# nelilepo/timetabling-ga-mpi-openmp

Hardware: AMD Instinct MI355X
Metric: fitness evals/sec (hcv+scv), pop 64K, 400-event instance; 1/2/4/8 GPUs (higher is better)
Workload: dtype i32; 1 GPU; med instance E=400 R=10 F=5 S=200 (seeded synthetic, medium01-size), population 65536 per GPU, one tt_eval (hcv+scv+feasible+penalty) per step; pop_per_gpu=65536, global_pop=65536, kernel=eval_tile5_w8, parallelism=dp1 (independent population shards)

## Files before the change

### timetabling-ga-mpi-openmp_amd/csrc/tt_eval.hip

```cpp
#include <algorithm>
#include <type_traits>
#include <utility>
#include <vector>

#include "tt_internal.h"

namespace ttga {

typedef __attribute__((address_space(4))) const uint32_t ConstU32;
typedef __attribute__((address_space(4))) const int32_t ConstI32;


__device__ __forceinline__ int bcnt_acc(uint32_t x, int acc) {
    int r;
    asm("v_bcnt_u32_b32 %0, %1, %2" : "=v"(r) : "v"(x), "v"(acc));
    return r;
}
__device__ __forceinline__ int popc_acc(uint64_t x, int acc) {
    int r, t;
    asm("v_bcnt_u32_b32 %0, %1, %2" : "=v"(t) : "v"((uint32_t)x), "v"(acc));
    asm("v_bcnt_u32_b32 %0, %1, %2" : "=v"(r) : "v"((uint32_t)(x >> 32)), "v"(t));
    return r;
}

__device__ __forceinline__ uint32_t lds_addr(const void* p) {
    return (uint32_t)(uintptr_t)(const __attribute__((address_space(3))) void*)p;
}
#define TT_RD(k, o) "ds_read_b64 %" #k ", %" #o " offset:" #k "*8\n"
template <int N>
__device__ __forceinline__ void lds_row_b64(uint32_t addr, uint64_t* v) {
    static_assert(N >= 1 && N <= 7, "1..7 words");
    uint64_t d[7];
    if constexpr (N == 7)
        asm volatile(TT_RD(0, 7) TT_RD(1, 7) TT_RD(2, 7) TT_RD(3, 7) TT_RD(4, 7) TT_RD(5, 7) TT_RD(6, 7) "s_waitcnt lgkmcnt(0)"
                     : "=&v"(d[0]), "=&v"(d[1]), "=&v"(d[2]), "=&v"(d[3]), "=&v"(d[4]), "=&v"(d[5]), "=&v"(d[6])
                     : "v"(addr) : "memory");
    else if constexpr (N == 6)
        asm volatile(TT_RD(0, 6) TT_RD(1, 6) TT_RD(2, 6) TT_RD(3, 6) TT_RD(4, 6) TT_RD(5, 6) "s_waitcnt lgkmcnt(0)"
                     : "=&v"(d[0]), "=&v"(d[1]), "=&v"(d[2]), "=&v"(d[3]), "=&v"(d[4]), "=&v"(d[5]) : "v"(addr) : "memory");
    else if constexpr (N == 5)
        asm volatile(TT_RD(0, 5) TT_RD(1, 5) TT_RD(2, 5) TT_RD(3, 5) TT_RD(4, 5) "s_waitcnt lgkmcnt(0)"
                     : "=&v"(d[0]), "=&v"(d[1]), "=&v"(d[2]), "=&v"(d[3]), "=&v"(d[4]) : "v"(addr) : "memory");
    else if constexpr (N == 4)
        asm volatile(TT_RD(0, 4) TT_RD(1, 4) TT_RD(2, 4) TT_RD(3, 4) "s_waitcnt lgkmcnt(0)"
                     : "=&v"(d[0]), "=&v"(d[1]), "=&v"(d[2]), "=&v"(d[3]) : "v"(addr) : "memory");
    else if constexpr (N == 3)
        asm volatile(TT_RD(0, 3) TT_RD(1, 3) TT_RD(2, 3) "s_waitcnt lgkmcnt(0)"
                     : "=&v"(d[0]), "=&v"(d[1]), "=&v"(d[2]) : "v"(addr) : "memory");
    else if constexpr (N == 2)
        asm volatile(TT_RD(0, 2) TT_RD(1, 2) "s_waitcnt lgkmcnt(0)" : "=&v"(d[0]), "=&v"(d[1]) : "v"(addr) : "memory");
    else
        asm volatile(TT_RD(0, 1) "s_waitcnt lgkmcnt(0)" : "=&v"(d[0]) : "v"(addr) : "memory");
#pragma unroll
    for (int k = 0; k < N; ++k) v[k] = d[k];
}
#undef TT_RD

#define TT_O(k) [d##k] "=&v"(d[k])
#define TT_I(k) [x##k] "v"(k < NA ? a : b), [o##k] "i"(k < NA ? 8 * k : 8 * (k - NA))
#define TT_R(k) "ds_read_b64 %[d" #k "], %[x" #k "] offset:%[o" #k "]\n"
template <int NA, int NB>
__device__ __forceinline__ void lds_two_rows(uint32_t a, uint32_t b, uint64_t* v) {
    constexpr int N = NA + NB;
    static_assert(NA >= 1 && NB >= 0 && N <= 8, "1..8 words");
    uint64_t d[8];
    if constexpr (N == 8)
        asm volatile(TT_R(0) TT_R(1) TT_R(2) TT_R(3) TT_R(4) TT_R(5) TT_R(6) TT_R(7) "s_waitcnt lgkmcnt(0)"
                     : TT_O(0), TT_O(1), TT_O(2), TT_O(3), TT_O(4), TT_O(5), TT_O(6), TT_O(7)
                     : TT_I(0), TT_I(1), TT_I(2), TT_I(3), TT_I(4), TT_I(5), TT_I(6), TT_I(7) : "memory");
    else if constexpr (N == 7)
        asm volatile(TT_R(0) TT_R(1) TT_R(2) TT_R(3) TT_R(4) TT_R(5) TT_R(6) "s_waitcnt lgkmcnt(0)"
                     : TT_O(0), TT_O(1), TT_O(2), TT_O(3), TT_O(4), TT_O(5), TT_O(6)
                     : TT_I(0), TT_I(1), TT_I(2), TT_I(3), TT_I(4), TT_I(5), TT_I(6) : "memory");
    else if constexpr (N == 6)
        asm volatile(TT_R(0) TT_R(1) TT_R(2) TT_R(3) TT_R(4) TT_R(5) "s_waitcnt lgkmcnt(0)"
                     : TT_O(0), TT_O(1), TT_O(2), TT_O(3), TT_O(4), TT_O(5)
                     : TT_I(0), TT_I(1), TT_I(2), TT_I(3), TT_I(4), TT_I(5) : "memory");
    else if constexpr (N == 5)
        asm volatile(TT_R(0) TT_R(1) TT_R(2) TT_R(3) TT_R(4) "s_waitcnt lgkmcnt(0)"
                     : TT_O(0), TT_O(1), TT_O(2), TT_O(3), TT_O(4) : TT_I(0), TT_I(1), TT_I(2), TT_I(3), TT_I(4) : "memory");
    else if constexpr (N == 4)
        asm volatile(TT_R(0) TT_R(1) TT_R(2) TT_R(3) "s_waitcnt lgkmcnt(0)"
                     : TT_O(0), TT_O(1), TT_O(2), TT_O(3) : TT_I(0), TT_I(1), TT_I(2), TT_I(3) : "memory");
    else if constexpr (N == 3)
        asm volatile(TT_R(0) TT_R(1) TT_R(2) "s_waitcnt lgkmcnt(0)"
                     : TT_O(0), TT_O(1), TT_O(2) : TT_I(0), TT_I(1), TT_I(2) : "memory");
    else if constexpr (N == 2)
        asm volatile(TT_R(0) TT_R(1) "s_waitcnt lgkmcnt(0)" : TT_O(0), TT_O(1) : TT_I(0), TT_I(1) : "memory");
    else
        asm volatile(TT_R(0) "s_waitcnt lgkmcnt(0)" : TT_O(0) : TT_I(0) : "memory");
#pragma unroll
    for (int k = 0; k < N; ++k) v[k] = d[k];
}
#undef TT_O
#undef TT_I
#undef TT_R

template <int R, int EWC>
__device__ __forceinline__ void corr_words(uint32_t bbase, const uint32_t* sv, const uint64_t (*cup)[EWC], int lane,
                                           int E, bool last_partial, int& h) {
    constexpr int S = EWC - 1 - R;
    if constexpr (R < S) {
        const uint32_t ss = (S < EWC - 1 || !last_partial || lane + 64 * S < E) ? sv[S] : 0u;
        uint64_t bw[EWC + 1];
        lds_two_rows<EWC - R, EWC - S>(bbase + sv[R] * (uint32_t)(EWC * 8) + 8 * R,
                                       bbase + ss * (uint32_t)(EWC * 8) + 8 * S, bw);
#pragma unroll
        for (int w = R; w < EWC; ++w) h = popc_acc(cup[R][w] & bw[w - R], h);
#pragma unroll
        for (int w = S; w < EWC; ++w) h = popc_acc(cup[S][w] & bw[EWC - R + w - S], h);
        corr_words<R + 1, EWC>(bbase, sv, cup, lane, E, last_partial, h);
    } else if constexpr (R == S) {
        if (R < EWC - 1 || !last_partial || lane + 64 * R < E) {
            uint64_t bw[EWC - R];
            lds_row_b64<EWC - R>(bbase + sv[R] * (uint32_t)(EWC * 8) + 8 * R, bw);
#pragma unroll
            for (int w = R; w < EWC; ++w) h = popc_acc(cup[R][w] & bw[w - R], h);
        }
    }
}

template <int ST>
__device__ __forceinline__ void sload_rec(const ConstU32* q, uint32_t (&r)[ST]) {
#pragma unroll
    for (int j = 0; j < ST; ++j) r[j] = q[j];
}
template <int ST>
__device__ __forceinline__ void keep_rec(const uint32_t (&r)[ST]) {
#pragma unroll
    for (int j = 0; j < ST; ++j) asm volatile("" ::"s"(r[j]));
}

constexpr uint32_t kGapLoK = 0x1FF7FDFFu, kGapLoG = 0x20080200u;
constexpr uint32_t kGapHiK = 0x0007FDFFu, kGapHiG = 0x00080200u;
__device__ __forceinline__ int mask_scv_gap(uint64_t m) {
    int sc = __popcll(m & (m >> 1) & (m >> 2));
    const uint32_t lo = (uint32_t)m, hi = (uint32_t)(m >> 32);
    const uint32_t blo = lo + kGapLoK, bhi = hi + kGapHiK;
    const uint32_t tlo = (lo & blo) + kGapLoK, thi = (hi & bhi) + kGapHiK;
    sc += __popc((blo ^ tlo) & kGapLoG);
    sc += __popc((bhi ^ thi) & kGapHiG);
    return sc;
}
__device__ __forceinline__ uint32_t gap_slots4(uint32_t x) {
    const uint32_t o = x | 0x80808080u;
    const uint32_t g9 = ((o - 0x09090909u) >> 7) & 0x01010101u, g18 = ((o - 0x12121212u) >> 7) & 0x01010101u;
    const uint32_t g27 = ((o - 0x1B1B1B1Bu) >> 7) & 0x01010101u, g36 = ((o - 0x24242424u) >> 7) & 0x01010101u;
    return x + g9 + g18 + g36 + 3u * g27;
}
__device__ __forceinline__ uint8_t gap_slot(uint32_t s) { return (uint8_t)gap_slots4(s); }
template <bool GAP>
__device__ __forceinline__ int mask_terms(uint64_t m) { return GAP ? mask_scv_gap(m) : mask_scv(m); }
template <int N, int K, bool GAP = false>
__device__ __forceinline__ int students_scv(const uint8_t* my, const uint32_t* r) {
    constexpr int H = N / 2;
    uint32_t sl[K * N];
#pragma unroll
    for (int k = 0; k < K; ++k)
#pragma unroll
        for (int j = 0; j < N; ++j) sl[k * N + j] = my[(r[k * H + (j >> 1)] >> (16 * (j & 1))) & 0xFFFFu];
    int sc = 0;
#pragma unroll
    for (int k = 0; k < K; ++k) {
        uint64_t m = 0;
#pragma unroll
        for (int j = 0; j < N; ++j) m |= 1ull << (sl[k * N + j] & 63);
        sc += mask_terms<GAP>(m);
    }
    return sc;
}
template <int N, int KMAX, bool GAP = false>
__device__ __forceinline__ int run_scv(const uint8_t* my, const uint32_t* p, int cnt) {
    constexpr int K = N <= 16 ? KMAX : 1;
    constexpr int ST = K * N / 2;
    const int steps = cnt / K;
    int sc = 0;
    if constexpr (KMAX == 1) {
        const ConstU32* q = (const ConstU32*)p;
        uint32_t cur[N / 2];
#pragma unroll
        for (int j = 0; j < N / 2; ++j) cur[j] = q[j];
        for (int i = 0; i < cnt; ++i) {
            const int in = i + 1 < cnt ? i + 1 : i;
            uint32_t nxt[N / 2];
#pragma unroll
            for (int j = 0; j < N / 2; ++j) nxt[j] = q[in * (N / 2) + j];
            uint32_t sl[N];
#pragma unroll
            for (int j = 0; j < N; ++j) sl[j] = my[(cur[j >> 1] >> (16 * (j & 1))) & 0xFFFFu];
            uint64_t m = 0;
#pragma unroll
            for (int j = 0; j < N; ++j) m |= 1ull << (sl[j] & 63);
            sc += mask_terms<GAP>(m);
#pragma unroll
            for (int j = 0; j < N / 2; ++j) cur[j] = nxt[j];
        }
        return sc;
    }
    const ConstU32* q = (const ConstU32*)p;
    if (steps > 0) {
        int i = 0;
        uint32_t ra[ST], rb[ST];
        sload_rec<ST>(q, ra);
        while (true) {
            sload_rec<ST>(q + (i + 1 < steps ? i + 1 : i) * ST, rb);
            sc += students_scv<N, K, GAP>(my, ra);
            keep_rec<ST>(rb);
            if (++i == steps) break;
            sload_rec<ST>(q + (i + 1 < steps ? i + 1 : i) * ST, ra);
            sc += students_scv<N, K, GAP>(my, rb);
            keep_rec<ST>(ra);
            if (++i == steps) break;
        }
    }
    if constexpr (K == 2) {
        if (cnt & 1) {
            uint32_t r[N / 2];
            sload_rec<N / 2>(q + steps * ST, r);
            sc += students_scv<N, 1, GAP>(my, r);
        }
    }
    return sc;
}
__device__ __noinline__ int run_scv_any(const uint8_t* my, const ConstU32* p, int cnt, int n, bool gap) {
    int sc = 0;
    for (int i = 0; i < cnt; ++i) {
        uint64_t m = 0;
        for (int j = 0; j < n / 2; ++j) {
            const uint32_t d = p[i * (n / 2) + j];
            m |= 1ull << (my[d & 0xFFFFu] & 63);
            m |= 1ull << (my[d >> 16] & 63);
        }
        sc += gap ? mask_scv_gap(m) : mask_scv(m);
    }
    return sc;
}
template <int KMAX, bool GAP = false>
__device__ __forceinline__ int lane_scv_runs(const uint8_t* my, const DevProblem& pb, int r0, int r1) {
    const ConstI32* runs = (const ConstI32*)pb.srun;
    int sc = 0;
    for (int k = r0; k < r1; ++k) {
        const int n = runs[4 * k], off = runs[4 * k + 1], cnt = runs[4 * k + 2];
        const uint32_t* p = pb.sid + off;
        switch (n) {
#define TT_RUN(N) case N: sc += run_scv<N, KMAX, GAP>(my, p, cnt); break;
            TT_RUN(2) TT_RUN(4) TT_RUN(6) TT_RUN(8) TT_RUN(10) TT_RUN(12) TT_RUN(14) TT_RUN(16)
            TT_RUN(18) TT_RUN(20) TT_RUN(22) TT_RUN(24) TT_RUN(26) TT_RUN(28) TT_RUN(30) TT_RUN(32)
#undef TT_RUN
            default: sc += run_scv_any(my, (const ConstU32*)p, cnt, n, GAP); break;
        }
    }
    return sc;
}

#ifndef TT_EVAL_ABLATE
#define TT_EVAL_ABLATE 0
#endif
__host__ __device__ inline int t5_cnt_bytes(int R) {
    return kSlots * ((R + 1) / 2) * 4;
}

struct Tile5Layout {
    int SP, WS;
    size_t tile_bytes, off_ws, off_part, bytes;
};

__host__ __device__ inline Tile5Layout tile5_layout(int E, int R, int NW, bool DB = false) {
    Tile5Layout L;
    int sp = (E + 1 + 3) & ~3;
    if (((sp >> 2) & 1) == 0) sp += 4;
    L.SP = sp;
    const int ew64 = (E + 63) / 64;
    const int cntb = t5_cnt_bytes(R);
    L.WS = (kSlots * ew64 * 8 + cntb + 15) & ~15;
    L.tile_bytes = ((size_t)64 * sp + 15) & ~(size_t)15;
    L.off_ws = (DB ? 2 : 1) * L.tile_bytes;
    L.off_part = L.off_ws + (size_t)NW * L.WS;
    L.bytes = L.off_part + 4 * (size_t)(NW * 64 + 64);
    return L;
}

template <int NW>
__device__ __forceinline__ void tile_dma(const uint8_t* src, uint8_t* dst, int np, int E, int SP, int wv, int lane) {
    const int qd = E >> 2;
    const __amdgpu_buffer_rsrc_t rs = __builtin_amdgcn_make_buffer_rsrc((void*)src, 0, np * E, 0x00020000);
    for (int r = wv; r < np; r += NW) {
        if (lane < qd)
            __builtin_amdgcn_raw_ptr_buffer_load_lds(rs, (__attribute__((address_space(3))) void*)(dst + r * SP), 4,
                                                     4 * lane, r * E, 0, 0);
        if (lane + 64 < qd)
            __builtin_amdgcn_raw_ptr_buffer_load_lds(rs, (__attribute__((address_space(3))) void*)(dst + r * SP + 256),
                                                     4, 4 * lane + 256, r * E, 0, 0);
    }
}

#ifdef TT_T5_STAMP
constexpr int kT5Launches = 8, kT5MaxBlocks = 16384, kT5Words = 10;
__device__ unsigned long long g_t5_stamp[kT5Launches * kT5MaxBlocks * kT5Words];
#endif

__device__ __forceinline__ uint32_t mad_u16_hi(uint32_t a, uint32_t b, uint32_t c) {
    uint32_t d;
    asm("v_mad_u32_u16 %0, %1, %2, %3 op_sel:[0,1,0,0]" : "=v"(d) : "v"(a), "v"(b), "v"(c));
    return d;
}

constexpr int kT5PrioLane = 3;
constexpr uint32_t kT5PrioW = 0x00112233u;
template <int EWC, int NW, int PK, bool DB = false>
__global__ __launch_bounds__(64 * NW, 4) void eval_tile5_kernel(DevProblem pb, const uint8_t* __restrict__ slot,
                                                              const uint8_t* __restrict__ room, int P,
                                                              int32_t* __restrict__ hcv_out,
                                                              int32_t* __restrict__ scv_out,
                                                              uint8_t* __restrict__ feas_out,
                                                              int32_t* __restrict__ pen_out, int ablate_arg) {
    extern __shared__ __attribute__((aligned(16))) uint8_t lds[];
    const int ablate = TT_EVAL_ABLATE ? ablate_arg : (ablate_arg & 3);
    constexpr int NT = 64 * NW;
#ifdef TT_T5_STAMP
    unsigned long long* st_rec =
        g_t5_stamp + ((size_t)((ablate_arg >> 8) & (kT5Launches - 1)) * kT5MaxBlocks + (blockIdx.x % kT5MaxBlocks)) * kT5Words;
    if (threadIdx.x == 0) {
        const unsigned long long t0 = __builtin_amdgcn_s_memrealtime();
        unsigned hw, xcc;
        asm volatile("s_getreg_b32 %0, hwreg(HW_REG_HW_ID)" : "=s"(hw));
        asm volatile("s_getreg_b32 %0, hwreg(HW_REG_XCC_ID)" : "=s"(xcc));
        st_rec[0] = t0;
        st_rec[1] = ((unsigned long long)xcc << 32) | hw;
    }
#endif
    const int E = pb.E, R = pb.R;
    const int lane = threadIdx.x & 63, wv = wave_id();
    const Tile5Layout L = tile5_layout(E, R, NW, DB);
    const int SP = L.SP;
    uint8_t* tile = lds;
    uint8_t* ws = lds + L.off_ws + (size_t)wv * L.WS;
    uint64_t* B = (uint64_t*)ws;
    uint32_t* cnt = (uint32_t*)(B + kSlots * EWC);
    int32_t* part = (int32_t*)(lds + L.off_part);
    int32_t* hq = part + NW * 64;
    const int tiles = (P + 63) / 64;
    const bool last_partial = E < 64 * EWC;
    const int RW = (R + 1) / 2;

    using PossT = typename std::conditional<PK == 0, uint64_t, uint32_t>::type;
    uint64_t inv_cup[EWC][EWC];
    PossT inv_poss[EWC];
    uint32_t inv_ps[EWC];
    int inv_sn[EWC];
#pragma unroll
    for (int r = 0; r < EWC; ++r) {
        const int e = lane + 64 * r;
        const bool ok = e < E;
        if constexpr (PK == 1) {
            inv_ps[r] = ok ? ((~(uint32_t)pb.poss[e] & 0xFFFFu) | ((uint32_t)pb.sn[e] << 16)) : 0u;
        } else {
            inv_poss[r] = ok ? (PossT)pb.poss[e] : (PossT)~0ull;
            inv_sn[r] = ok ? pb.sn[e] : 0;
        }
#pragma unroll
        for (int w = 0; w < EWC; ++w) inv_cup[r][w] = (w >= r && ok) ? pb.cupT[(size_t)w * E + e] : 0ull;
    }
    const ConstI32* ptab = (const ConstI32*)pb.srun_part;
    const int pbase = srun_part_base(NW);
    const int r0 = ptab[pbase + wv], r1 = ptab[pbase + wv + 1];
    const bool wide = (E & 15) == 0 && (((uintptr_t)slot) & 15) == 0;
    const int qpr = E >> 4;
    const uint32_t qinv = ((1u << 20) + (uint32_t)qpr - 1) / (uint32_t)max(qpr, 1);

    if constexpr (DB) {
        if (threadIdx.x < 128) lds[(threadIdx.x >> 6) * L.tile_bytes + (threadIdx.x & 63) * SP + E] = 63;
        if (blockIdx.x < tiles)
            tile_dma<NW>(slot + (long)blockIdx.x * 64 * E, lds, (int)min(64L, (long)P - (long)blockIdx.x * 64), E, SP,
                         wv, lane);
    }
    int it = 0;
    for (int tl = blockIdx.x; tl < tiles; tl += gridDim.x, ++it) {
        const long p0 = (long)tl * 64;
        const int np = (int)min((long)64, (long)P - p0);
        const uint8_t* src = slot + p0 * E;
        if constexpr (DB) {
            tile = lds + (it & 1) * L.tile_bytes;
            asm volatile("s_waitcnt vmcnt(0)" ::: "memory");
            __syncthreads();
            const int tn = tl + gridDim.x;
            if (tn < tiles)
                tile_dma<NW>(slot + (long)tn * 64 * E, lds + ((it + 1) & 1) * L.tile_bytes,
                             (int)min(64L, (long)P - (long)tn * 64), E, SP, wv, lane);
        } else {
        __syncthreads();
        if (wide) {
            const uint4* s16 = (const uint4*)src;
#pragma unroll 2
            for (int w = threadIdx.x; w < np * qpr; w += NT) {
                const int r = (int)(((uint32_t)w * qinv) >> 20), c = w - r * qpr;
                const uint4 v = s16[w];
                uint32_t* d = (uint32_t*)(tile + r * SP + 16 * c);
                d[0] = v.x; d[1] = v.y; d[2] = v.z; d[3] = v.w;
            }
        } else {
#pragma unroll 1
            for (int r = wv; r < np; r += NW)
#pragma unroll 1
                for (int c = lane; c < E; c += 64) tile[r * SP + c] = src[(long)r * E + c];
        }
        if (threadIdx.x < 64) tile[threadIdx.x * SP + E] = 63;
        __syncthreads();
        }

        uint32_t lsp;
        asm volatile("v_mul_u32_u24 %0, %1, %2" : "=v"(lsp) : "v"(lane), "s"(SP));
        __builtin_amdgcn_s_setprio(kT5PrioLane);
        const int sc = (!(ablate & 1) && r0 < r1) ? lane_scv_runs<1>(tile + lsp, pb, r0, r1) : 0;
        part[wv * 64 + lane] = sc;

        const int nq = (ablate & 2) ? 0 : np;
        uint32_t pfn[EWC];
        const __amdgpu_buffer_rsrc_t rrs =
            __builtin_amdgcn_make_buffer_rsrc((void*)(room + p0 * E), 0, 64 * E, 0x00020000);
        auto load_row = [&](int q, uint32_t* dst) {
#pragma unroll
            for (int r = 0; r < EWC; ++r)
                dst[r] = (!last_partial || r < EWC - 1 || lane + 64 * r < E)
                             ? (uint32_t)__builtin_amdgcn_raw_buffer_load_b8(rrs, lane + 64 * r, q * E, 0)
                             : 0u;
        };
        if (wv < nq) load_row(wv, pfn);
        for (int q = wv; q < nq; q += NW) {
            const uint32_t pr = (kT5PrioW >> (4 * min((q - wv) / NW, 7))) & 3u;
            if (pr == 0) __builtin_amdgcn_s_setprio(0);
            else if (pr == 1) __builtin_amdgcn_s_setprio(1);
            else if (pr == 2) __builtin_amdgcn_s_setprio(2);
            else __builtin_amdgcn_s_setprio(3);
            uint32_t rv[EWC], sv[EWC];
#pragma unroll
            for (int r = 0; r < EWC; ++r) rv[r] = pfn[r];
            const uint8_t* rs = tile + q * SP;
#pragma unroll
            for (int r = 0; r < EWC; ++r)
                sv[r] = (!last_partial || r < EWC - 1 || lane + 64 * r < E) ? rs[lane + 64 * r] : 0u;
            if (q + NW < nq) load_row(q + NW, pfn);
            uint32_t smax = 0, rmax = 0;
#pragma unroll
            for (int r = 0; r < EWC; ++r) { smax = max(smax, sv[r]); rmax = max(rmax, rv[r]); }
            const bool any_bad = wave_any(smax >= (uint32_t)kSlots || rmax >= (uint32_t)R);
            int h = 0, last = 0;
            if (!any_bad) {
                if (!(ablate & 32))
                    for (int c = lane; c < (L.WS >> 4); c += 64) ((uint4*)ws)[c] = make_uint4(0u, 0u, 0u, 0u);
                __builtin_amdgcn_fence(__ATOMIC_RELEASE, "wavefront");
                __builtin_amdgcn_wave_barrier();
                __builtin_amdgcn_fence(__ATOMIC_ACQUIRE, "wavefront");
#pragma unroll
                for (int r = 0; r < EWC; ++r) {
                    if (r < EWC - 1 || !last_partial || lane + 64 * r < E) {
                        const uint32_t s = sv[r], ro = rv[r];
                        if (!(ablate & 8)) atomicOr((unsigned long long*)&B[s * EWC + r], 1ull << lane);
                        if (!(ablate & 16)) {
                            uint32_t* c = (uint32_t*)((uint8_t*)cnt + ((__umul24(s, (uint32_t)(2 * RW)) + (ro & ~1u)) << 1));
                            const uint32_t sh = ro << 4;
                            h += (int)__builtin_amdgcn_ubfe(atomicAdd(c, 1u << (sh & 31u)), sh, 16);
                        }
                        const bool last_slot = (kLastSlotMask >> s) & 1ull;
                        if constexpr (PK == 1) {
                            h += (int)__builtin_amdgcn_ubfe(inv_ps[r], ro, 1);
                            last = (int)mad_u16_hi((uint32_t)(kLastSlotMask >> s) & 1u, inv_ps[r], (uint32_t)last);
                        } else {
                            h += (int)(((inv_poss[r] >> ro) & 1u) ^ 1u);
                            last += last_slot ? inv_sn[r] : 0;
                        }
                    }
                }
                __builtin_amdgcn_fence(__ATOMIC_RELEASE, "wavefront");
                __builtin_amdgcn_wave_barrier();
                __builtin_amdgcn_fence(__ATOMIC_ACQUIRE, "wavefront");
                if (!(ablate & 4)) {
                    corr_words<0, EWC>(lds_addr(B), sv, inv_cup, lane, E, last_partial, h);
                }
                if (!wave_any(h >= 1024 || last >= 1024)) {
                    const uint32_t t = (uint32_t)wave_sum((h << 16) | last);
                    h = (int)(t >> 16);
                    last = (int)(t & 0xFFFFu);
                } else {
                    h = wave_sum(h);
                    last = wave_sum(last);
                }
                __builtin_amdgcn_fence(__ATOMIC_RELEASE, "wavefront");
                __builtin_amdgcn_wave_barrier();
                __builtin_amdgcn_fence(__ATOMIC_ACQUIRE, "wavefront");
            }
            if (lane == 0) {
                hq[q] = any_bad ? -1 : h;
                part[wv * 64 + q] += last;
            }
        }
        __syncthreads();
        if (wv == 0 && lane < np) {
            const long p = p0 + lane;
            const int h = hq[lane];
            if (h < 0) {
                hcv_out[p] = -1; scv_out[p] = -1; feas_out[p] = 0; pen_out[p] = -1;
            } else {
                int s2 = 0;
#pragma unroll
                for (int w = 0; w < NW; ++w) s2 += part[w * 64 + lane];
                hcv_out[p] = h;
                scv_out[p] = s2;
                feas_out[p] = h == 0 ? 1 : 0;
                pen_out[p] = h == 0 ? s2 : 1000000 + h;
            }
        }
    }
#ifdef TT_T5_STAMP
    if ((threadIdx.x & 63) == 0 && (threadIdx.x >> 6) < kT5Words - 2)
        st_rec[2 + (threadIdx.x >> 6)] = __builtin_amdgcn_s_memrealtime();
#endif
}

template <int NWL>
__global__ __launch_bounds__(64 * NWL) void eval_lanes_kernel(DevProblem pb, const uint8_t* __restrict__ slot, int P,
                                                              int32_t* __restrict__ scv_part) {
    extern __shared__ __attribute__((aligned(16))) uint8_t lds[];
    constexpr int NT = 64 * NWL;
    const int E = pb.E;
    const int lane = threadIdx.x & 63, wv = wave_id();
    int sp = (E + 1 + 3) & ~3;
    if (((sp >> 2) & 1) == 0) sp += 4;
    const int SP = sp;
    uint8_t* tile = lds;
    int32_t* part = (int32_t*)(lds + (((size_t)64 * SP + 15) & ~(size_t)15));
    const int tiles = (P + 63) / 64;
    const ConstI32* ptab = (const ConstI32*)pb.srun_part;
    const int pbase = srun_part_base(NWL);
    const int r0 = ptab[pbase + wv], r1 = ptab[pbase + wv + 1];
    const bool wide = (E & 15) == 0 && (((uintptr_t)slot) & 15) == 0;
    const int qpr = E >> 4;
    const uint64_t qinv = ((1ull << 32) + (uint64_t)qpr - 1) / (uint64_t)max(qpr, 1);

    for (int tl = blockIdx.x; tl < tiles; tl += gridDim.x) {
        const long p0 = (long)tl * 64;
        const int np = (int)min((long)64, (long)P - p0);
        __syncthreads();
        const uint8_t* src = slot + p0 * E;
        if (wide) {
            const uint4* s16 = (const uint4*)src;
#pragma unroll 2
            for (int w = threadIdx.x; w < np * qpr; w += NT) {
                const int r = (int)(((uint64_t)(uint32_t)w * qinv) >> 32), c = w - r * qpr;
                const uint4 v = s16[w];
                uint32_t* d = (uint32_t*)(tile + r * SP + 16 * c);
                d[0] = gap_slots4(v.x); d[1] = gap_slots4(v.y); d[2] = gap_slots4(v.z); d[3] = gap_slots4(v.w);
            }
        } else {
#pragma unroll 1
            for (int r = wv; r < np; r += NWL)
#pragma unroll 1
                for (int c = lane; c < E; c += 64) {
                    const uint8_t v = src[(long)r * E + c];
                    tile[r * SP + c] = gap_slot(v);
                }
        }
        if (threadIdx.x < 64) tile[threadIdx.x * SP + E] = 63;
        __syncthreads();
        const int sc = r0 < r1 ? lane_scv_runs<2, true>(tile + lane * SP, pb, r0, r1) : 0;
        part[wv * 64 + lane] = sc;
        __syncthreads();
        if (wv == 0 && lane < np) {
            int s2 = 0;
#pragma unroll
            for (int w = 0; w < NWL; ++w) s2 += part[w * 64 + lane];
            scv_part[p0 + lane] = s2;
        }
    }
}

struct CorrLayout {
    int NWV, BST, NB, EPL;
    size_t off_cnt, off_sl, WSI, off_acc, off_red, bytes;
};

__host__ __device__ inline CorrLayout corr_layout(int E, int R, int EW64, int NB) {
    CorrLayout L;
    const int pairs = (EW64 + 1) / 2;
    L.NWV = pairs < 16 ? pairs : 16;
    L.EPL = (E + 64 * L.NWV - 1) / (64 * L.NWV);
    L.BST = EW64 | 1;
    L.off_cnt = (size_t)kSlots * L.BST * 8;
    L.off_sl = L.off_cnt + (size_t)((kSlots * R + 1) / 2) * 4;
    L.WSI = (L.off_sl + (size_t)E + 15) & ~(size_t)15;
    L.NB = NB;
    L.off_acc = (size_t)NB * L.WSI;
    L.off_red = L.off_acc + (size_t)NB * 16;
    L.bytes = L.off_red + (size_t)NB * 2 * 64 * 4;
    return L;
}

constexpr int kCorrMaxEPL = 4;

template <int N, int OFF>
__device__ __forceinline__ void lds_gather(const uint32_t* a, uint64_t* v) {
    static_assert(N == 2 || N == 4 || N == 8, "2, 4 or 8 reads");
    if constexpr (N == 8)
        asm volatile("ds_read_b64 %0, %8 offset:%16\n ds_read_b64 %1, %9 offset:%16\n ds_read_b64 %2, %10 offset:%16\n"
                     "ds_read_b64 %3, %11 offset:%16\n ds_read_b64 %4, %12 offset:%16\n ds_read_b64 %5, %13 offset:%16\n"
                     "ds_read_b64 %6, %14 offset:%16\n ds_read_b64 %7, %15 offset:%16\n s_waitcnt lgkmcnt(0)"
                     : "=&v"(v[0]), "=&v"(v[1]), "=&v"(v[2]), "=&v"(v[3]), "=&v"(v[4]), "=&v"(v[5]), "=&v"(v[6]), "=&v"(v[7])
                     : "v"(a[0]), "v"(a[1]), "v"(a[2]), "v"(a[3]), "v"(a[4]), "v"(a[5]), "v"(a[6]), "v"(a[7]), "i"(OFF)
                     : "memory");
    else if constexpr (N == 4)
        asm volatile("ds_read_b64 %0, %4 offset:%8\n ds_read_b64 %1, %5 offset:%8\n ds_read_b64 %2, %6 offset:%8\n"
                     "ds_read_b64 %3, %7 offset:%8\n s_waitcnt lgkmcnt(0)"
                     : "=&v"(v[0]), "=&v"(v[1]), "=&v"(v[2]), "=&v"(v[3])
                     : "v"(a[0]), "v"(a[1]), "v"(a[2]), "v"(a[3]), "i"(OFF) : "memory");
    else
        asm volatile("ds_read_b64 %0, %2 offset:%4\n ds_read_b64 %1, %3 offset:%4\n s_waitcnt lgkmcnt(0)"
                     : "=&v"(v[0]), "=&v"(v[1]) : "v"(a[0]), "v"(a[1]), "i"(OFF) : "memory");
}

template <int NB>
__device__ __forceinline__ void corr_chunk(const DevProblem& pb, int c, int lane, const uint32_t (&r)[NB], int (&h)[NB]) {
    const int E = pb.E, EW = pb.EW64, e = 64 * c + lane;
    const bool ev = e < E;
    const uint64_t* src = pb.cupT + (ev ? e : 0);
    uint64_t x[4];
#pragma unroll
    for (int j = 0; j < 4; ++j) x[j] = (ev && c + j < EW) ? src[(size_t)(c + j) * E] : 0ull;
    for (int w = c; w < EW; w += 4) {
        uint64_t y[4];
#pragma unroll
        for (int j = 0; j < 4; ++j) y[j] = (ev && w + 4 + j < EW) ? src[(size_t)(w + 4 + j) * E] : 0ull;
        uint32_t b[NB];
#pragma unroll
        for (int q = 0; q < NB; ++q) b[q] = r[q] + 8u * (uint32_t)w;
        [&]<int... J>(std::integer_sequence<int, J...>) {
            ([&] {
                if (w + J < EW) {
                    uint64_t v[NB];
                    lds_gather<NB, 8 * J>(b, v);
#pragma unroll
                    for (int q = 0; q < NB; ++q) h[q] = popc_acc(x[J] & v[q], h[q]);
                }
            }(), ...);
        }(std::make_integer_sequence<int, 4>{});
#pragma unroll
        for (int j = 0; j < 4; ++j) x[j] = y[j];
    }
}

template <int NB, int MEPL>
__global__ __launch_bounds__(1024) void eval_corr_kernel(DevProblem pb, const uint8_t* __restrict__ slot,
                                                         const uint8_t* __restrict__ room, int P,
                                                         int32_t* __restrict__ hcv_out, int32_t* __restrict__ scv_io,
                                                         uint8_t* __restrict__ feas_out, int32_t* __restrict__ pen_out,
                                                         int ablate_arg) {
    extern __shared__ __attribute__((aligned(16))) uint8_t lds[];
    const int ablate = TT_EVAL_ABLATE ? ablate_arg : (ablate_arg & 3);
    const int E = pb.E, R = pb.R, EW = pb.EW64;
    const CorrLayout L = corr_layout(E, R, EW, NB);
    const int lane = threadIdx.x & 63, wv = wave_id();
    const int NWV = L.NWV, pairs = (EW + 1) / 2, EPL = L.EPL;
    const uint32_t WSI = (uint32_t)L.WSI, BSTB = (uint32_t)L.BST * 8u;
    int32_t* acc = (int32_t*)(lds + L.off_acc);
    int32_t* red = (int32_t*)(lds + L.off_red);
    const uint32_t lds0 = lds_addr(lds);

    const int eb = (wv * 64 + lane) * EPL;
    const bool pair16 = EPL == 2 && (E & 1) == 0 && (((uintptr_t)slot | (uintptr_t)room) & 1) == 0;
    uint64_t possv[MEPL];
    int snv[MEPL];
#pragma unroll
    for (int j = 0; j < MEPL; ++j) {
        const bool ok = j < EPL && eb + j < E;
        possv[j] = ok ? pb.poss[eb + j] : ~0ull;
        snv[j] = ok ? pb.sn[eb + j] : 0;
    }

    const long batches = ((long)P + NB - 1) / NB;
    for (long bt = blockIdx.x; bt < batches; bt += gridDim.x) {
        const long q0 = bt * NB;
        const int nq = (int)min((long)NB, (long)P - q0);
        __syncthreads();
        for (int i = threadIdx.x; i < (int)(L.bytes >> 4); i += blockDim.x)
            ((uint4*)lds)[i] = make_uint4(0u, 0u, 0u, 0u);
        __syncthreads();
        if (!(ablate & 1)) {
            uint32_t svq[NB], rvq[NB];
#pragma unroll
            for (int q = 0; q < NB; ++q) {
                svq[q] = 0u; rvq[q] = 0u;
                if (q < nq) {
                    const uint8_t* srow = slot + (q0 + q) * E + eb;
                    const uint8_t* rrow = room + (q0 + q) * E + eb;
                    if (pair16 && eb + 1 < E) {
                        svq[q] = *(const uint16_t*)srow;
                        rvq[q] = *(const uint16_t*)rrow;
                    } else {
#pragma unroll
                        for (int j = 0; j < MEPL; ++j)
                            if (j < EPL && eb + j < E) {
                                svq[q] |= (uint32_t)srow[j] << (8 * j);
                                rvq[q] |= (uint32_t)rrow[j] << (8 * j);
                            }
                    }
                }
            }
#pragma unroll
            for (int q = 0; q < NB; ++q) {
                if (q >= nq) break;
                const uint32_t sv = svq[q], rv = rvq[q];
                uint8_t* wsq = lds + (size_t)q * WSI;
                uint64_t* B = (uint64_t*)wsq;
                uint32_t* cnt = (uint32_t*)(wsq + L.off_cnt);
                int h = 0, last = 0;
                bool bad = false;
#pragma unroll
                for (int j = 0; j < MEPL; ++j) {
                    const int e = eb + j;
                    if (j < EPL && e < E) {
                        const uint32_t s = (sv >> (8 * j)) & 0xFFu, ro = (rv >> (8 * j)) & 0xFFu;
                        wsq[L.off_sl + e] = (uint8_t)min(s, (uint32_t)kSlots - 1);
                        if (s >= (uint32_t)kSlots || ro >= (uint32_t)R) {
                            bad = true;
                        } else {
                            atomicOr((unsigned long long*)&B[s * (uint32_t)L.BST + (uint32_t)(e >> 6)], 1ull << (e & 63));
                            const uint32_t cell = s * (uint32_t)R + ro, sh = (cell & 1u) << 4;
                            h += (int)((atomicAdd(&cnt[cell >> 1], 1u << sh) >> sh) & 0xFFFFu);
                            h += (int)(((possv[j] >> ro) & 1ull) ^ 1ull);
                            last += ((kLastSlotMask >> s) & 1ull) ? snv[j] : 0;
                        }
                    }
                }
                atomicAdd(&red[(2 * q) * 64 + lane], h);
                atomicAdd(&red[(2 * q + 1) * 64 + lane], last);
                if (wave_any(bad) && lane == 0) atomicOr(&acc[4 * q + 2], 1);
            }
        }
        __syncthreads();
        if (!(ablate & 2)) {
            for (int pr = wv; pr < pairs; pr += NWV) {
                const int ca = pr, cb = EW - 1 - pr;
                int hq[NB];
#pragma unroll
                for (int q = 0; q < NB; ++q) hq[q] = 0;
#pragma unroll
                for (int side = 0; side < 2; ++side) {
                    const int c = side ? cb : ca;
                    if (side && cb == ca) break;
                    const int e = 64 * c + lane;
                    uint32_t r[NB];
#pragma unroll
                    for (int q = 0; q < NB; ++q) {
                        const uint32_t sq = (q < nq && e < E) ? (uint32_t)lds[(size_t)q * WSI + L.off_sl + e] : 0u;
                        r[q] = lds0 + (q < nq ? q : 0) * WSI + sq * BSTB;
                    }
                    corr_chunk<NB>(pb, c, lane, r, hq);
                }
#pragma unroll
                for (int q = 0; q < NB; ++q) {
                    if (q >= nq) break;
                    atomicAdd(&red[(2 * q) * 64 + lane], hq[q]);
                }
            }
        }
        __syncthreads();
        for (int k = wv; k < 2 * nq; k += NWV) {
            const int v = wave_sum(red[k * 64 + lane]);
            if (lane == 0) acc[4 * (k >> 1) + (k & 1)] = v;
        }
        __syncthreads();
        if (threadIdx.x < nq) {
            const long q = q0 + threadIdx.x;
            const int* a = acc + 4 * threadIdx.x;
            if (a[2]) {
                hcv_out[q] = -1; scv_io[q] = -1; feas_out[q] = 0; pen_out[q] = -1;
            } else {
                const int h = a[0], s2 = scv_io[q] + a[1];
                hcv_out[q] = h;
                scv_io[q] = s2;
                feas_out[q] = h == 0 ? 1 : 0;
                pen_out[q] = h == 0 ? s2 : 1000000 + h;
            }
        }
    }
}

static size_t lanes_lds_bytes(int E) {
    int sp = (E + 1 + 3) & ~3;
    if (((sp >> 2) & 1) == 0) sp += 4;
    return (((size_t)64 * sp + 15) & ~(size_t)15) + 4 * (size_t)16 * 64;
}

constexpr size_t kCorrLdsBudget = 152 * 1024;

static int corr_nb(int E, int R, int EW64) {
    for (int nb = 8; nb >= 2; nb >>= 1)
        if (corr_layout(E, R, EW64, nb).bytes <= kCorrLdsBudget) return nb;
    return 0;
}

constexpr int kBlockThreads = 256;

__global__ __launch_bounds__(kBlockThreads) void eval_block_kernel(DevProblem pb, const uint8_t* __restrict__ slot,
                                                                   const uint8_t* __restrict__ room, int P,
                                                                   int32_t* __restrict__ hcv_out,
                                                                   int32_t* __restrict__ scv_out,
                                                                   uint8_t* __restrict__ feas_out,
                                                                   int32_t* __restrict__ pen_out) {
    extern __shared__ __attribute__((aligned(16))) uint8_t lds[];
    const int E = pb.E, R = pb.R, S = pb.S, EW = pb.EW;
    const int tid = threadIdx.x;
    const long p = blockIdx.x;
    const int cells = kSlots * R;
    uint32_t* cnt = (uint32_t*)lds;
    uint32_t* bcnt = cnt + cells;
    uint32_t* bstart = bcnt + kSlots;
    uint32_t* bcur = bstart + kSlots;
    int32_t* red = (int32_t*)(bcur + kSlots);
    uint16_t* bucket = (uint16_t*)(red + 4);
    uint8_t* sl = (uint8_t*)(bucket + ((E + 1) & ~1));

    const uint8_t* gs = slot + p * E;
    const uint8_t* gr = room + p * E;
    for (int c = tid; c < cells; c += kBlockThreads) cnt[c] = 0u;
    for (int c = tid; c < kSlots; c += kBlockThreads) { bcnt[c] = 0u; bcur[c] = 0u; }
    if (tid < 4) red[tid] = 0;
    for (int e = tid; e < E; e += kBlockThreads) sl[e] = gs[e];
    __syncthreads();

    int h = 0, sc = 0;
    bool bad = false;
    for (int e = tid; e < E; e += kBlockThreads) {
        const int s = sl[e], r = gr[e];
        if (s >= kSlots || r >= R) { bad = true; continue; }
        h += (int)atomicAdd(&cnt[s * R + r], 1u);
        h += ((pb.poss[e] >> r) & 1ull) ? 0 : 1;
        sc += ((kLastSlotMask >> s) & 1ull) ? pb.sn[e] : 0;
        atomicAdd(&bcnt[s], 1u);
    }
    if (bad) atomicOr(&red[2], 1);
    __syncthreads();
    if (tid == 0) {
        uint32_t acc = 0;
        for (int t = 0; t < kSlots; ++t) { bstart[t] = acc; acc += bcnt[t]; }
    }
    __syncthreads();
    if (red[2] == 0) {
        for (int e = tid; e < E; e += kBlockThreads) {
            const int s = sl[e];
            bucket[bstart[s] + atomicAdd(&bcur[s], 1u)] = (uint16_t)e;
        }
    }
    __syncthreads();
    if (red[2] == 0) {
        for (int i = tid; i < E; i += kBlockThreads) {
            const int s = sl[i];
            const uint32_t* row = pb.corr + (size_t)i * EW;
            const uint32_t b0 = bstart[s], b1 = b0 + bcnt[s];
            for (uint32_t b = b0; b < b1; ++b) {
                const int j = bucket[b];
                if (j > i) h += (row[j >> 5] >> (j & 31)) & 1u;
            }
        }
        for (int st = tid; st < S; st += kBlockThreads) {
            uint64_t m = 0;
            for (int k = pb.stu_off[st]; k < pb.stu_off[st + 1]; ++k) m |= 1ull << sl[pb.stu_ev[k]];
            sc += __popcll(m & (m >> 1) & (m >> 2) & kTripleMask);
#pragma unroll
            for (int d = 0; d < 5; ++d) sc += (__popc((uint32_t)(m >> (9 * d)) & 0x1FFu) == 1);
        }
    }
    h = wave_sum(h);
    sc = wave_sum(sc);
    if ((tid & 63) == 0) { atomicAdd(&red[0], h); atomicAdd(&red[1], sc); }
    __syncthreads();
    if (tid == 0) {
        if (red[2]) {
            hcv_out[p] = -1; scv_out[p] = -1; feas_out[p] = 0; pen_out[p] = -1;
        } else {
            const int hh = red[0], ss = red[1];
            hcv_out[p] = hh;
            scv_out[p] = ss;
            feas_out[p] = hh == 0 ? 1 : 0;
            pen_out[p] = hh == 0 ? ss : 1000000 + hh;
        }
    }
}

static size_t block_lds_bytes(int E, int R) {
    return 4 * (size_t)(kSlots * R + 3 * kSlots + 4) + 2 * (size_t)((E + 1) & ~1) + (size_t)E;
}

}

using namespace ttga;

static bool tile5_fits(const tt_problem* p, int NW) {
    return p->dev.EW64 <= 7 && p->E <= 32767 && tile5_layout(p->E, p->R, NW).bytes <= (NW == 8 ? 80 : 160) * 1024;
}

static bool wide_fits(const tt_problem* p) {
    const int EW64 = p->dev.EW64;
    return p->E <= 32767 && lanes_lds_bytes(p->E) <= 160 * 1024 &&
           corr_nb(p->E, p->R, EW64) > 0 && corr_layout(p->E, p->R, EW64, 2).EPL <= kCorrMaxEPL;
}

static int auto_variant(const tt_problem* p) {
    if (tile5_fits(p, 8)) return 8;
    if (tile5_fits(p, 4)) return 7;
    if (wide_fits(p)) return 13;
    return 2;
}

extern "C" int tt_eval_auto_variant(const tt_problem* p) { return p ? auto_variant(p) : -1; }

#ifdef TT_T5_STAMP
extern "C" int tt_t5_stamp_read(unsigned long long* out, int reset) {
    TT_HIP(hipDeviceSynchronize());
    TT_HIP(hipMemcpyFromSymbol(out, HIP_SYMBOL(g_t5_stamp), sizeof(g_t5_stamp)));
    if (reset) {
        std::vector<unsigned long long> z(sizeof(g_t5_stamp) / 8, 0ull);
        TT_HIP(hipMemcpyToSymbol(HIP_SYMBOL(g_t5_stamp), z.data(), sizeof(g_t5_stamp)));
    }
    return kT5Launches * kT5MaxBlocks;
}
#endif

extern "C" int tt_eval_variant(const tt_problem* p, const uint8_t* slot, const uint8_t* room, int P, int32_t* hcv,
                               int32_t* scv, uint8_t* feasible, int32_t* penalty, int variant, void* stream) {
    int rc = check_pop_args(p, P, slot, room);
    if (rc) return rc;
    if (P > 0 && (!hcv || !scv || !feasible || !penalty)) { set_error("null output buffer"); return TT_ERR_INVALID; }
    const int ablate = variant >> 4;
    variant &= 15;
    if (variant != 0 && variant != 2 && variant != 7 && variant != 8 && variant != 13) {
        set_error("unknown eval variant (0 auto, 2 block, 7/8 tile5, 13 wide)");
        return TT_ERR_INVALID;
    }
    if (P == 0) return TT_OK;
    rc = use_device(p);
    if (rc) return rc;
    hipStream_t st = (hipStream_t)stream;
    const int E = p->E, R = p->R;
    if (variant == 0) variant = auto_variant(p);
    if (variant == 13) {
        if (!wide_fits(p)) { set_error("instance outside the wide eval path"); return TT_ERR_LIMIT; }
        const int EW64 = p->dev.EW64;
        const int tiles = (P + 63) / 64;
        {
            const size_t lds_l = lanes_lds_bytes(E);
            auto launch_l = [&](auto kern) -> int {
                int per_cu = 0;
                TT_HIP(hipOccupancyMaxActiveBlocksPerMultiprocessor(&per_cu, kern, 1024, lds_l));
                per_cu = std::min(per_cu, lds_resident_limit(lds_l));
                const int grid = std::min(tiles, std::max(1, per_cu) * p->num_cus);
                hipLaunchKernelGGL(kern, dim3(grid), dim3(1024), lds_l, st, p->dev, slot, P, scv);
                return TT_OK;
            };
            rc = launch_l(eval_lanes_kernel<16>);
            if (rc) return rc;
        }
        if (ablate & 4) return check_hip(hipGetLastError(), "tt_eval launch");
        const int NB = corr_nb(E, R, EW64);
        const CorrLayout CL = corr_layout(E, R, EW64, NB);
        auto launch = [&](auto kern) -> int {
            int per_cu = 0;
            TT_HIP(hipOccupancyMaxActiveBlocksPerMultiprocessor(&per_cu, kern, 64 * CL.NWV, CL.bytes));
            per_cu = std::min(per_cu, lds_resident_limit(CL.bytes));
            const long batches = ((long)P + NB - 1) / NB;
            const int grid = (int)std::min<long>(batches, (long)std::max(1, per_cu) * p->num_cus);
            hipLaunchKernelGGL(kern, dim3(grid), dim3(64 * CL.NWV), CL.bytes, st, p->dev, slot, room, P, hcv, scv,
                               feasible, penalty, ablate);
            return TT_OK;
        };
        if (CL.EPL <= 2)
            rc = NB == 8 ? launch(eval_corr_kernel<8, 2>) : NB == 4 ? launch(eval_corr_kernel<4, 2>) : launch(eval_corr_kernel<2, 2>);
        else
            rc = NB == 8 ? launch(eval_corr_kernel<8, kCorrMaxEPL>)
                 : NB == 4 ? launch(eval_corr_kernel<4, kCorrMaxEPL>) : launch(eval_corr_kernel<2, kCorrMaxEPL>);
        if (rc) return rc;
    } else if (variant == 7 || variant == 8) {
        const int NW = variant == 7 ? 4 : 8;
        const Tile5Layout L0 = tile5_layout(E, R, NW, false), L1 = tile5_layout(E, R, NW, true);
        const bool db_ok = (E & 3) == 0 && (((uintptr_t)slot) & 3) == 0 && L1.bytes <= 160 * 1024;
        if (p->dev.EW64 > 7 || L0.bytes > 160 * 1024 || E > 32767) {
            set_error("instance too large for the tile5 kernel");
            return TT_ERR_LIMIT;
        }
        const int max_sn = p->max_sn;
        const int pk = (R <= 16 && max_sn <= 0xFFFF) ? 1 : R <= 32 ? 2 : 0;
        const int tiles = (P + 63) / 64;
        auto occupancy = [&](auto kern, size_t bytes, bool two) -> int {
            std::atomic<int>& c = const_cast<tt_problem*>(p)->t5_occ[NW == 8][two];
            int per_cu = c.load(std::memory_order_relaxed);
            if (per_cu >= 0) return per_cu;
            if (hipOccupancyMaxActiveBlocksPerMultiprocessor(&per_cu, kern, 64 * NW, bytes) != hipSuccess) {
                (void)hipGetLastError();
                return 0;
            }
            per_cu = std::min(per_cu, lds_resident_limit(bytes));
            c.store(per_cu, std::memory_order_relaxed);
            return per_cu;
        };
        auto launch = [&](auto kern, size_t bytes, bool two) -> int {
            const int per_cu = occupancy(kern, bytes, two);
            const bool persist = (ablate & 64) || (two && !(ablate & 128));
            const int grid = persist ? std::min(tiles, std::max(1, per_cu) * p->num_cus) : tiles;
            hipLaunchKernelGGL(kern, dim3(grid), dim3(64 * NW), bytes, st, p->dev, slot, room, P, hcv, scv,
                               feasible, penalty, ablate);
            return TT_OK;
        };
#define TT_T5U(EWC, NWV, PKV)                                                                                      \
    {                                                                                                              \
        const bool db = db_ok && occupancy(eval_tile5_kernel<EWC, NWV, PKV, true>, L1.bytes, true) >=              \
                                     occupancy(eval_tile5_kernel<EWC, NWV, PKV, false>, L0.bytes, false);          \
        rc = db ? launch(eval_tile5_kernel<EWC, NWV, PKV, true>, L1.bytes, true)                                   \
                : launch(eval_tile5_kernel<EWC, NWV, PKV, false>, L0.bytes, false);                                \
    }
#define TT_T5N(EWC, NWV) \
    if (pk == 1) { TT_T5U(EWC, NWV, 1) } else if (pk == 2) { TT_T5U(EWC, NWV, 2) } else { TT_T5U(EWC, NWV, 0) }
#define TT_T5(EWC)                                                      \
    case EWC:                                                           \
        if (NW == 4) { TT_T5N(EWC, 4) } else { TT_T5N(EWC, 8) }         \
        break;
        switch (p->dev.EW64) {
            TT_T5(1) TT_T5(2) TT_T5(3) TT_T5(4) TT_T5(5) TT_T5(6) TT_T5(7)
            default: rc = TT_ERR_LIMIT; break;
        }
#undef TT_T5
#undef TT_T5N
#undef TT_T5U
        if (rc) return rc;
    } else {
        const size_t lds = block_lds_bytes(E, R);
        if (lds > 160 * 1024) { set_error("instance too large for the block kernel"); return TT_ERR_LIMIT; }
        hipLaunchKernelGGL(eval_block_kernel, dim3(P), dim3(kBlockThreads), lds, st, p->dev, slot, room, P, hcv,
                           scv, feasible, penalty);
    }
    return check_hip(hipGetLastError(), "tt_eval launch");
}

extern "C" int tt_eval(const tt_problem* p, const uint8_t* slot, const uint8_t* room, int P, int32_t* hcv,
                       int32_t* scv, uint8_t* feasible, int32_t* penalty, void* stream) {
    return tt_eval_variant(p, slot, room, P, hcv, scv, feasible, penalty, 0, stream);
}
```

Before: 949.2 million evals/s.

## Clear per-wave LDS workspace via computed-jump ds_write_addtid and precompute row addresses

Replaces the per-lane uint4 zeroing loop of the wave workspace with an inline-asm computed jump into an unrolled run of ds_write_addtid_b32 stores using M0 as the base, with a biased path for workspaces above 64KB. Row base addresses for each slot are computed once and reused by both the bitmask atomicOr and the correlation reads. The partial-lane guards in corr_words are dropped, so inactive lanes read row 0 of the slot matrix. The aim is fewer VALU and address instructions per individual. In exchange it adds fragile PC-relative assembly and new layout-reach limits on which instances tile5 accepts.

```diff
diff --git a/timetabling-ga-mpi-openmp_amd/csrc/tt_eval.hip b/timetabling-ga-mpi-openmp_amd/csrc/tt_eval.hip
--- a/timetabling-ga-mpi-openmp_amd/csrc/tt_eval.hip
+++ b/timetabling-ga-mpi-openmp_amd/csrc/tt_eval.hip
@@ -9,6 +9,7 @@
 
 typedef __attribute__((address_space(4))) const uint32_t ConstU32;
 typedef __attribute__((address_space(4))) const int32_t ConstI32;
+typedef __attribute__((address_space(3))) unsigned long long LdsU64;
 
 
 __device__ __forceinline__ int bcnt_acc(uint32_t x, int acc) {
@@ -26,40 +27,10 @@
 __device__ __forceinline__ uint32_t lds_addr(const void* p) {
     return (uint32_t)(uintptr_t)(const __attribute__((address_space(3))) void*)p;
 }
-#define TT_RD(k, o) "ds_read_b64 %" #k ", %" #o " offset:" #k "*8\n"
-template <int N>
-__device__ __forceinline__ void lds_row_b64(uint32_t addr, uint64_t* v) {
-    static_assert(N >= 1 && N <= 7, "1..7 words");
-    uint64_t d[7];
-    if constexpr (N == 7)
-        asm volatile(TT_RD(0, 7) TT_RD(1, 7) TT_RD(2, 7) TT_RD(3, 7) TT_RD(4, 7) TT_RD(5, 7) TT_RD(6, 7) "s_waitcnt lgkmcnt(0)"
-                     : "=&v"(d[0]), "=&v"(d[1]), "=&v"(d[2]), "=&v"(d[3]), "=&v"(d[4]), "=&v"(d[5]), "=&v"(d[6])
-                     : "v"(addr) : "memory");
-    else if constexpr (N == 6)
-        asm volatile(TT_RD(0, 6) TT_RD(1, 6) TT_RD(2, 6) TT_RD(3, 6) TT_RD(4, 6) TT_RD(5, 6) "s_waitcnt lgkmcnt(0)"
-                     : "=&v"(d[0]), "=&v"(d[1]), "=&v"(d[2]), "=&v"(d[3]), "=&v"(d[4]), "=&v"(d[5]) : "v"(addr) : "memory");
-    else if constexpr (N == 5)
-        asm volatile(TT_RD(0, 5) TT_RD(1, 5) TT_RD(2, 5) TT_RD(3, 5) TT_RD(4, 5) "s_waitcnt lgkmcnt(0)"
-                     : "=&v"(d[0]), "=&v"(d[1]), "=&v"(d[2]), "=&v"(d[3]), "=&v"(d[4]) : "v"(addr) : "memory");
-    else if constexpr (N == 4)
-        asm volatile(TT_RD(0, 4) TT_RD(1, 4) TT_RD(2, 4) TT_RD(3, 4) "s_waitcnt lgkmcnt(0)"
-                     : "=&v"(d[0]), "=&v"(d[1]), "=&v"(d[2]), "=&v"(d[3]) : "v"(addr) : "memory");
-    else if constexpr (N == 3)
-        asm volatile(TT_RD(0, 3) TT_RD(1, 3) TT_RD(2, 3) "s_waitcnt lgkmcnt(0)"
-                     : "=&v"(d[0]), "=&v"(d[1]), "=&v"(d[2]) : "v"(addr) : "memory");
-    else if constexpr (N == 2)
-        asm volatile(TT_RD(0, 2) TT_RD(1, 2) "s_waitcnt lgkmcnt(0)" : "=&v"(d[0]), "=&v"(d[1]) : "v"(addr) : "memory");
-    else
-        asm volatile(TT_RD(0, 1) "s_waitcnt lgkmcnt(0)" : "=&v"(d[0]) : "v"(addr) : "memory");
-#pragma unroll
-    for (int k = 0; k < N; ++k) v[k] = d[k];
-}
-#undef TT_RD
-
 #define TT_O(k) [d##k] "=&v"(d[k])
-#define TT_I(k) [x##k] "v"(k < NA ? a : b), [o##k] "i"(k < NA ? 8 * k : 8 * (k - NA))
+#define TT_I(k) [x##k] "v"(k < NA ? a : b), [o##k] "i"(k < NA ? OA + 8 * k : OB + 8 * (k - NA))
 #define TT_R(k) "ds_read_b64 %[d" #k "], %[x" #k "] offset:%[o" #k "]\n"
-template <int NA, int NB>
+template <int NA, int NB, int OA, int OB>
 __device__ __forceinline__ void lds_two_rows(uint32_t a, uint32_t b, uint64_t* v) {
     constexpr int N = NA + NB;
     static_assert(NA >= 1 && NB >= 0 && N <= 8, "1..8 words");
@@ -97,26 +68,21 @@
 #undef TT_R
 
 template <int R, int EWC>
-__device__ __forceinline__ void corr_words(uint32_t bbase, const uint32_t* sv, const uint64_t (*cup)[EWC], int lane,
-                                           int E, bool last_partial, int& h) {
+__device__ __forceinline__ void corr_words(const uint32_t* row, const uint64_t (*cup)[EWC], int& h) {
     constexpr int S = EWC - 1 - R;
     if constexpr (R < S) {
-        const uint32_t ss = (S < EWC - 1 || !last_partial || lane + 64 * S < E) ? sv[S] : 0u;
         uint64_t bw[EWC + 1];
-        lds_two_rows<EWC - R, EWC - S>(bbase + sv[R] * (uint32_t)(EWC * 8) + 8 * R,
-                                       bbase + ss * (uint32_t)(EWC * 8) + 8 * S, bw);
+        lds_two_rows<EWC - R, EWC - S, 8 * R, 8 * S>(row[R], row[S], bw);
 #pragma unroll
         for (int w = R; w < EWC; ++w) h = popc_acc(cup[R][w] & bw[w - R], h);
 #pragma unroll
         for (int w = S; w < EWC; ++w) h = popc_acc(cup[S][w] & bw[EWC - R + w - S], h);
-        corr_words<R + 1, EWC>(bbase, sv, cup, lane, E, last_partial, h);
+        corr_words<R + 1, EWC>(row, cup, h);
     } else if constexpr (R == S) {
-        if (R < EWC - 1 || !last_partial || lane + 64 * R < E) {
-            uint64_t bw[EWC - R];
-            lds_row_b64<EWC - R>(bbase + sv[R] * (uint32_t)(EWC * 8) + 8 * R, bw);
-#pragma unroll
-            for (int w = R; w < EWC; ++w) h = popc_acc(cup[R][w] & bw[w - R], h);
-        }
+        uint64_t bw[EWC - R];
+        lds_two_rows<EWC - R, 0, 8 * R, 0>(row[R], row[R], bw);
+#pragma unroll
+        for (int w = R; w < EWC; ++w) h = popc_acc(cup[R][w] & bw[w - R], h);
     }
 }
 
@@ -303,6 +269,39 @@
     uint32_t d;
     asm("v_mad_u32_u16 %0, %1, %2, %3 op_sel:[0,1,0,0]" : "=v"(d) : "v"(a), "v"(b), "v"(c));
     return d;
+}
+
+constexpr uint32_t kT5ClrBias = 0x8000u;
+constexpr size_t kT5ClrReach = 0x10000u + kT5ClrBias;
+constexpr int t5_clear_max(int EWC, int PK) {
+    return (kSlots * EWC * 8 + kSlots * (PK == 1 ? 8 : PK == 2 ? 16 : 32) * 4 + 15) / 256;
+}
+template <int MAXF>
+__device__ __forceinline__ void t5_clear_pieces(uint32_t m0v, uint32_t skip) {
+    uint32_t keep;
+    asm volatile("s_mov_b32 %[keep], m0\n"
+                 "s_mov_b32 m0, %[base]\n"
+                 "s_getpc_b64 vcc\n"
+                 "s_add_u32 vcc_lo, vcc_lo, %[skip]\n"
+                 "s_addc_u32 vcc_hi, vcc_hi, 0\n"
+                 "s_setpc_b64 vcc\n"
+                 ".set tt_clr_k, %c[n]\n"
+                 ".rept %c[n]\n"
+                 ".set tt_clr_k, tt_clr_k-1\n"
+                 "ds_write_addtid_b32 %[z] offset:tt_clr_k*256\n"
+                 ".endr\n"
+                 "s_branch .Ltt_clr_end%=\n"
+                 ".set tt_clr_k, %c[n]\n"
+                 ".rept %c[n]\n"
+                 ".set tt_clr_k, tt_clr_k-1\n"
+                 "ds_write_addtid_b32 %[z] offset:tt_clr_k*256+%c[bias]\n"
+                 ".endr\n"
+                 ".Ltt_clr_end%=:\n"
+                 "s_mov_b32 m0, %[keep]\n"
+                 "s_nop 0"
+                 : [keep] "=&s"(keep)
+                 : [base] "s"(m0v), [skip] "s"(skip), [z] "v"(0u), [n] "i"(MAXF), [bias] "i"(kT5ClrBias)
+                 : "memory", "scc", "vcc");
 }
 
 constexpr int kT5PrioLane = 3;
@@ -342,6 +341,11 @@
     const int tiles = (P + 63) / 64;
     const bool last_partial = E < 64 * EWC;
     const int RW = (R + 1) / 2;
+    constexpr int CLRF = t5_clear_max(EWC, PK);
+    const uint32_t ws_a = (uint32_t)__builtin_amdgcn_readfirstlane((int)lds_addr(ws));
+    const bool ws_hi = ws_a >= 0x10000u;
+    const uint32_t clr_m0 = ws_hi ? ws_a - kT5ClrBias : ws_a;
+    const uint32_t clr_skip = 12u + 8u * (uint32_t)(CLRF - min(L.WS >> 8, CLRF)) + (ws_hi ? 8u * CLRF + 4u : 0u);
 
     using PossT = typename std::conditional<PK == 0, uint64_t, uint32_t>::type;
     uint64_t inv_cup[EWC][EWC];
@@ -446,8 +450,13 @@
             const bool any_bad = wave_any(smax >= (uint32_t)kSlots || rmax >= (uint32_t)R);
             int h = 0, last = 0;
             if (!any_bad) {
-                if (!(ablate & 32))
-                    for (int c = lane; c < (L.WS >> 4); c += 64) ((uint4*)ws)[c] = make_uint4(0u, 0u, 0u, 0u);
+                uint32_t row[EWC];
+#pragma unroll
+                for (int r = 0; r < EWC; ++r) row[r] = lds_addr(B) + __umul24(sv[r], (uint32_t)(EWC * 8));
+                if (!(ablate & 32)) {
+                    t5_clear_pieces<CLRF>(clr_m0, clr_skip);
+                    *(uint32_t*)(ws + L.WS - 256 + 4 * lane) = 0u;
+                }
                 __builtin_amdgcn_fence(__ATOMIC_RELEASE, "wavefront");
                 __builtin_amdgcn_wave_barrier();
                 __builtin_amdgcn_fence(__ATOMIC_ACQUIRE, "wavefront");
@@ -455,7 +464,9 @@
                 for (int r = 0; r < EWC; ++r) {
                     if (r < EWC - 1 || !last_partial || lane + 64 * r < E) {
                         const uint32_t s = sv[r], ro = rv[r];
-                        if (!(ablate & 8)) atomicOr((unsigned long long*)&B[s * EWC + r], 1ull << lane);
+                        if (!(ablate & 8))
+                            __hip_atomic_fetch_or((LdsU64*)(uintptr_t)row[r] + r, 1ull << lane, __ATOMIC_RELAXED,
+                                                  __HIP_MEMORY_SCOPE_AGENT);
                         if (!(ablate & 16)) {
                             uint32_t* c = (uint32_t*)((uint8_t*)cnt + ((__umul24(s, (uint32_t)(2 * RW)) + (ro & ~1u)) << 1));
                             const uint32_t sh = ro << 4;
@@ -475,7 +486,7 @@
                 __builtin_amdgcn_wave_barrier();
                 __builtin_amdgcn_fence(__ATOMIC_ACQUIRE, "wavefront");
                 if (!(ablate & 4)) {
-                    corr_words<0, EWC>(lds_addr(B), sv, inv_cup, lane, E, last_partial, h);
+                    corr_words<0, EWC>(row, inv_cup, h);
                 }
                 if (!wave_any(h >= 1024 || last >= 1024)) {
                     const uint32_t t = (uint32_t)wave_sum((h << 16) | last);
@@ -895,7 +906,8 @@
 using namespace ttga;
 
 static bool tile5_fits(const tt_problem* p, int NW) {
-    return p->dev.EW64 <= 7 && p->E <= 32767 && tile5_layout(p->E, p->R, NW).bytes <= (NW == 8 ? 80 : 160) * 1024;
+    return p->dev.EW64 <= 7 && p->E <= 32767 && tile5_layout(p->E, p->R, NW).bytes <= (NW == 8 ? 80 : 160) * 1024 &&
+           tile5_layout(p->E, p->R, NW, true).off_part <= kT5ClrReach;
 }
 
 static bool wide_fits(const tt_problem* p) {
@@ -981,8 +993,9 @@
     } else if (variant == 7 || variant == 8) {
         const int NW = variant == 7 ? 4 : 8;
         const Tile5Layout L0 = tile5_layout(E, R, NW, false), L1 = tile5_layout(E, R, NW, true);
-        const bool db_ok = (E & 3) == 0 && (((uintptr_t)slot) & 3) == 0 && L1.bytes <= 160 * 1024;
-        if (p->dev.EW64 > 7 || L0.bytes > 160 * 1024 || E > 32767) {
+        const bool db_ok = (E & 3) == 0 && (((uintptr_t)slot) & 3) == 0 && L1.bytes <= 160 * 1024 &&
+                           L1.off_part <= kT5ClrReach;
+        if (p->dev.EW64 > 7 || L0.bytes > 160 * 1024 || L0.off_part > kT5ClrReach || E > 32767) {
             set_error("instance too large for the tile5 kernel");
             return TT_ERR_LIMIT;
         }
```

Measured after the change: 983.1 million evals/s, median of 6. +3.6%, better.
